# jlko/STOVE

Hardware: AMD Instinct MI355X
Metric: frames/s (fwd+bwd) for 3-obj billiards 32x32 T=100, 1/2/4/8 GPU; ELBO delta vs ref (higher is better)
Workload: dtype f32 (encoder GEMMs: fp32 products as 3 sixteen-bit MFMAs on hi/lo-split operands -- half pieces forward, bf16 pieces backward -- fp32 accumulate)

## Files before the change

### include/stove_hip.h

```cpp
#ifndef STOVE_HIP_H
#define STOVE_HIP_H
#include <stddef.h>
#include <stdint.h>

#ifdef __cplusplus
extern "C" {
#endif

int stove_abi_version(void);
const char* stove_error_string(int code);

typedef struct StoveSpnTables {
  const int32_t* obj_scope;
  const int32_t* obj_leaf_slot;
  const float* obj_coef;
  const float* obj_wsum;
  const float* obj_wroot;
  const int32_t* bg_side;
  const float* bg_coef;
  const float* bg_wroot;
  const float* bg_dense;
} StoveSpnTables;

size_t stove_bg_dense_floats(void);
// ... 255 lines not shown
int stove_supair_state_fwd2(const float* codes, const float* span_low, float* zc, float* pos, long long* idx, float* zfix,
                            unsigned char* hits, float* zl, float* sl, float* init, int init_ld, const float* lat_noise, int lat_dim,
                            int n, int T, int o, int skip, int fix, int mode, void* stream);
int stove_supair_state_bwd2(const float* zc, const long long* idx, const unsigned char* hits, const float* zfix, const float* g_zfix,
                            const float* g_zl, const float* g_sl, const float* g_init6, int init_ld, const float* span_low, float* gfix_ws,
                            float* g_codes, int n, int T, int o, int skip, void* stream);
int stove_zall_fwd(const float* zfix, const float* zs, float* zall, int n, int T, int o, int skip, void* stream);
int stove_zall_bwd(const float* zfix, const float* zs, const float* g_zall, const float* dz_in, float* g_zfix, float* g_zs, int n, int T, int o,
                   int skip, void* stream);
int stove_elbo_fwd(const float* zs, const float* mean, const float* std_, const float* zdyn, const float* lik, const float* trans_std16,
                   float* part_ws, float* out3, int n, int T, int o, int skip, void* stream);
int stove_elbo_bwd(const float* zs, const float* mean, const float* std_, const float* zdyn, const float* trans_std16, const float* g_out,
                   float* g_zs, float* g_mean, float* g_std, float* g_zdyn, float* g_lik, int n, int T, int o, int skip, void* stream);

void stove_debug_set_stamps(long long* device_buffer);

typedef struct StoveSpnArenaPlan {
  const int32_t* obj_mu;
  const int32_t* obj_rho;
  const int32_t* obj_sum;
  const int32_t* bg_mu;
  const int32_t* bg_rho;
  const int32_t* bg_gidx;
  int32_t obj_root, bg_root;
  float obj_vmin, obj_vmax, bg_vmin, bg_vmax;
} StoveSpnArenaPlan;
int stove_spn_bake(const float* arena, const StoveSpnArenaPlan* plan, float* obj_coef, float* obj_wsum, float* obj_wroot,
                   float* bg_coef, float* bg_wroot, void* stream);
int stove_spn_bake_bwd(const float* arena, const StoveSpnArenaPlan* plan, const StoveSpnTableGrads* g, float* grad_arena, void* stream);
int stove_arena_gather(const float* arena, const int32_t* src, float* image, int n, void* stream);
// ... 59 lines not shown
```

### stove_amd/_lib.py

```python
import ctypes
import os
from ctypes import POINTER, Structure, c_char_p, c_float, c_int, c_size_t, c_void_p

import torch

_HERE = os.path.dirname(os.path.abspath(__file__))
from . import settings as _settings

LIB_PATH = _settings.LIB_OVERRIDE or os.path.join(_HERE, 'libstove_hip.so')
_lib = None
ABI_VERSION = 7

class SpnTables(Structure):
    _fields_ = [('obj_scope', c_void_p), ('obj_leaf_slot', c_void_p), ('obj_coef', c_void_p),
                ('obj_wsum', c_void_p), ('obj_wroot', c_void_p),
                ('bg_side', c_void_p), ('bg_coef', c_void_p), ('bg_wroot', c_void_p), ('bg_dense', c_void_p)]


class SpnTableGrads(Structure):
    _fields_ = [('obj_coef', c_void_p), ('obj_wsum', c_void_p), ('obj_wroot', c_void_p),
                ('bg_coef', c_void_p), ('bg_wroot', c_void_p)]


class SpnArenaPlan(Structure):
# ... 85 lines not shown
        'stove_gnn_fwd_cl': (I, [P, P, P, P, I, I, I, I, I, I, P]),
        'stove_gnn_bwd_cl': (I, [P, P, P, P, P, P, P, I, I, I, I, I, I, P]),
        'stove_dynloop_fwd_cl': (I, [P] * 12 + [I] * 7 + [F] * 3 + [P]),
        'stove_dynloop_bwd_cl': (I, [P] * 18 + [I] * 7 + [F] * 3 + [P]),
        'stove_rollout_fwd_cl': (I, [P] * 6 + [I] * 8 + [F] * 3 + [P]),
        'stove_rollout_sample_fwd_cl': (I, [P] * 8 + [I] * 8 + [F] * 3 + [P]),
        'stove_match_objects': (I, [P, P, P, I, I, I, I, I, P]),
        'stove_profile_enable': (None, [I]),
        'stove_lstm_cell_fwd': (I, [P, P, P, P, P, I, I, I, P]),
        'stove_lstm_cell_bwd': (I, [P] * 10 + [I, I, I, I, P]),
        'stove_gnn_debug_stamps': (I, [P, P, P, P, P, P, I, I, I, I, I, P]),
        'stove_profile_report': (S, [c_char_p, S]),
        'stove_spn_bake': (I, [P, A, P, P, P, P, P, P]),
        'stove_spn_bake_bwd': (I, [P, A, G, P, P]),
        'stove_debug_set_stamps': (None, [P]),
        'stove_glimpse_mean': (I, [P, P, P, I, I, I, P]),
        'stove_objspn_mpe': (I, [T, P, P, P, P, P, I, P]),
        'stove_render_frames': (I, [P, P, I, P, P, I, I, P]),
        'stove_render_frames_any': (I, [P, P, I, P, P, P, P] + [I] * 8 + [P]),
        'stove_enc_head_fwd': (I, [P, P, P, P, P, P, P, I, I, I, I, I, I, P]),
        'stove_enc_head_bwd_ws_floats': (S, [I, I]),
        'stove_enc_head_bwd': (I, [P, P, P, P, P, P, P, P, P, P, I, P, I, I, I, I, I, P]),
        'stove_colsum2': (I, [P, P, P, I, P, I, I, P]),
        'stove_small_tn_ws_floats': (S, [I, I, I]),
        'stove_small_tn': (I, [P, P, P, P, I, I, I, P]),
        'stove_dynloop_bwd_ws_bytes_ts': (S, [I, I, I]),
        'stove_bw_transform': (I, [P, P, I, I, I, P]),
        'stove_bw_transform_u8': (I, [P, P, I, I, I, P]),
        'stove_stream_after': (I, [P, P]),
        'stove_small_linear': (I, [P, P, P, P, I, I, I, I, P]),
# ... 110 lines not shown
```

### stove_amd/csrc/capi.hip

```cpp
#include "../../include/stove_hip.h"
#include <algorithm>

#include "common.h"
#include <string.h>
#include <stdlib.h>
#include <math.h>
#include <atomic>
#include <type_traits>
#include "validate.h"
static_assert(stove_validate::kStoveInvalidValue == (int)hipErrorInvalidValue, "validate.h returns hipErrorInvalidValue");
#define STOVE_VALIDATE(expr)                      \
  do {                                            \
    const int v__ = stove_validate::expr;         \
    if (v__) return v__;                          \
  } while (0)
#include "spn_obj.hip"
#include "spn_obj_generic.hip"
#include "spn_bg.hip"
#include "spn_bg_generic.hip"
#include "scene.hip"
#include "scene_fused.hip"
#include "scene_colour.hip"
#include "gnn.hip"
#include "match.hip"
// ... 793 lines not shown
}

static long long* g_sm_stamps = nullptr;
void stove_debug_set_stamps(long long* device_buffer) { g_sm_stamps = device_buffer; }

size_t stove_dynloop_act_floats(int B, int Ts, int N) {
  const int g = gnn_group_for(B, N);
  const size_t blockwise = (size_t)stove_gnn_blocks(B, N) * Ts * gnn_act_floats(N, g);
  if (small_graph(N)) {
    const size_t streams = (size_t)B * sm_act2_floats(N, Ts);
    return streams > blockwise ? streams : blockwise;
  }
  return blockwise;
}

int stove_dynloop_fwd(const float* z1, const float* zsup, const float* zsstd, const float* eps, const float* extra,
                      const float* params, float* z, float* zdyn, float* zdstd, float* mean, float* std_, float* pred, float* act,
                      int B, int Ts, int N, int sin_dim, int lim_enc, int elu, float pos_var, float vel_std, float lat_std,
                      void* stream) {
  STOVE_VALIDATE(dynloop_fwd(z1, zsup, zsstd, eps, extra, params, z, zdyn, zdstd, mean, std_, B, Ts, N, sin_dim));
  if (B == 0 || Ts == 0) return 0;
  LoopConst kc{pos_var, vel_std, lat_std};
  if (small_graph(N)) {
    auto launch = [&](auto save, auto nmx, auto e, auto nt, auto stamp) {
      constexpr int NMX = decltype(nmx)::value;
      return STOVE_LAUNCH_LDS((dyn_loop_fwd_small_k<decltype(save)::value, NMX, decltype(e)::value, decltype(nt)::value, decltype(stamp)::value>),
                              dim3(B), dim3(64 * kSmWaves), SmShape<NMX>::kLdsFloats * sizeof(float), (hipStream_t)stream, z1, zsup, zsstd, eps,
                              extra, params, z, zdyn, zdstd, mean, std_, pred, act, B, Ts, N, sin_dim, lim_enc, elu, kc, g_sm_stamps, 0, Ts);
    };
    if (g_sm_stamps != nullptr && act != nullptr && !elu && N == 3)
      return launch(Int<2>{}, Int<4>{}, std::false_type{}, Int<3>{}, std::true_type{});
    auto run = [&](auto save) {
      return with_small_graph<true>(N, elu, true, [&](auto nmx, auto e, auto nt) { return launch(save, nmx, e, nt, std::false_type{}); });
    };
    return act != nullptr ? run(Int<2>{}) : run(Int<0>{});
  }
  const int G = gnn_group_for(B, N);
  return with_flag(elu, [&](auto e) {
    return with_flag(N == 6 && G == 1, [&](auto n6) {
      return STOVE_LAUNCH_LDS((dyn_loop_fwd_k<decltype(e)::value, decltype(n6)::value>), dim3(stove_gnn_blocks(B, N)), dim3(256), kGnnLdsBytes,
                              (hipStream_t)stream, z1, zsup, zsstd, eps, extra, params, z, zdyn, zdstd, mean, std_, pred, act, B, Ts, N, G,
                              sin_dim, lim_enc, elu, kc);
    });
// ... 19 lines not shown
                                   dextra, g_params, ws, B, Ts, N, sin_dim, lim_enc, elu, pos_var, vel_std, lat_std, stream, stream);
}

int stove_dynloop_bwd_overlap(const float* z1, const float* zsup, const float* zsstd, const float* eps, const float* extra,
                              const float* params, const float* z, const float* act, const float* dz, const float* dzdyn,
                              const float* dmean, const float* dstd, const float* dpred, float* dz1, float* dzsup, float* dzsstd,
                              float* dextra, float* g_params, void* ws, int B, int Ts, int N, int sin_dim, int lim_enc, int elu,
                              float pos_var, float vel_std, float lat_std, void* stream, void* param_stream) {
  STOVE_VALIDATE(dynloop_bwd(z1, zsup, zsstd, eps, extra, params, z, dz1, dzsup, dzsstd, dextra, g_params, ws, B, Ts, N, sin_dim));
  hipStream_t st = (hipStream_t)stream;
  hipStream_t sp = param_stream != nullptr ? (hipStream_t)param_stream : st;
  LoopConst kc{pos_var, vel_std, lat_std};
  if (small_bwd_path(N, act)) {
    float* gpart = (float*)ws;
    float* dy = gpart + (size_t)B * kGnnGrads;
    const bool head = dz != nullptr && dzdyn != nullptr && dmean != nullptr && dstd != nullptr && dpred == nullptr && sin_dim == 16 && lim_enc == 2;
    auto launch = [&](auto nmx, auto e, auto nt, auto hd, auto stamp) {
      constexpr int NMX = decltype(nmx)::value;
      return STOVE_LAUNCH_LDS((dyn_loop_bwd_small_k<NMX, decltype(e)::value, decltype(nt)::value, decltype(hd)::value, decltype(stamp)::value>),
                              dim3(B), dim3(64 * kSmWaves), smb_lds_floats<NMX>() * sizeof(float), st, zsup, zsstd, eps, params,
                              const_cast<float*>(act), dz, dzdyn, dmean, dstd, dpred, dz1, dzsup, dzsstd, dextra, dy, B, Ts, N, sin_dim, lim_enc,
                              elu, kc, g_sm_stamps, 0, Ts, (float*)nullptr);
    };
    int rc;
    if (g_sm_stamps != nullptr && !elu && N == 3 && head) {
      rc = launch(Int<4>{}, std::false_type{}, Int<3>{}, std::true_type{}, std::true_type{});
    } else {
      rc = with_small_graph<true>(N, elu, head, [&](auto nmx, auto e, auto nt) {
        constexpr int NT = decltype(nt)::value;
        if constexpr (NT == 6) {
          return launch(nmx, e, nt, std::true_type{}, std::false_type{});
        } else {
          if constexpr (NT == 3) {
            if (head) return launch(nmx, e, nt, std::true_type{}, std::false_type{});
          }
          return launch(nmx, e, nt, std::false_type{}, std::false_type{});
        }
      });
    }
    if (rc) return rc;
    STOVE_TRY(stream_after(sp, st));
    rc = STOVE_LAUNCH_LDS(gnn_dw_small_k, dim3(B), dim3(256), kDwLdsFloats * sizeof(float), sp, act, (const float*)dy, gpart, B, Ts, N);
    if (rc) return rc;
    STOVE_LAUNCH(reduce_chunks_k, dim3((kGnnGrads + 31) / 32), dim3(256), 0, sp, (const float*)gpart, g_params, kGnnGrads, B, 0);
    STOVE_LAUNCH_CHECK();
    return 0;
  }
  const int nb = stove_gnn_blocks(B, N), G = gnn_group_for(B, N);
  int rc = with_flag(elu, [&](auto e) {
    return with_flag(N == 6 && G == 1, [&](auto n6) {
      return STOVE_LAUNCH_LDS((dyn_loop_bwd_k<decltype(e)::value, decltype(n6)::value>), dim3(nb), dim3(256), kGnnLdsBytes, st, z1, zsup, zsstd,
                              eps, extra, params, z, act, dz, dzdyn, dmean, dstd, dpred, dz1, dzsup, dzsstd, dextra, (float*)ws, B, Ts, N, G,
                              sin_dim, lim_enc, elu, kc);
    });
  });
// ... 1136 lines not shown
```

### stove_amd/csrc/gnn_small.hip

```cpp
#include "common.h"
#include "split16.h"

namespace stove {

constexpr int kSmW = W_END;
constexpr int kSmWaves = 4;

template <int NMX>
struct SmShape {
  static_assert(NMX == 4 || NMX == 6, "built for up to four or up to six objects");
  static constexpr int RP = NMX > 4 ? 2 : 1;
  static constexpr int ET = (NMX * (NMX - 1) + 15) / 16;
  static constexpr int NE = NMX * NMX;
  static constexpr int kLdsFloats = kSmW + V_END + NMX * 256 + NMX * 4 + NE * 32 + ((NE + 3) & ~3);
};

struct SmLds {
  float *W, *V, *PR, *POS, *R3, *ATT;
};
template <int NMX>
__device__ __forceinline__ SmLds sm_carve(float* base) {
  SmLds L;
  L.W = base;
  L.V = L.W + kSmW;
// ... 487 lines not shown
    }
    sm_mfma_layer<2>(ws1, h1, acc);
    if (el[0].valid) {
#pragma unroll
      for (int t = 0; t < 2; ++t) {
        sm_st4(sdx + el[0].node32 + 16 * t, acc[t] + h1[t]);
        if (SAVE) sm_st4(act.H1 + el[0].node32 + 16 * t, h1[t]);
      }
    }
    return;
  }
  if ((wv != 2 && wv != 3) || cf.N < 2) return;
  sm_edge_chain<SAVE, ET>(L, cf, act, el, pre, cw, wv == 2 ? 1 : 0);
}

template <bool SAVE, int NMX>
__device__ __forceinline__ void sm_step(const SmLds& L, const SmCfg& cf, float sinv, const SmAct& act, float& res_out, float& pred_out,
                                        const SmEdgeLane (&el)[SmShape<NMX>::ET], const SmChainW& cw) {
  constexpr int RP = SmShape<NMX>::RP, ET = SmShape<NMX>::ET;
  constexpr bool HK = RP == 1;
  __shared__ __attribute__((aligned(16))) float sbuf[NMX][32];
  __shared__ __attribute__((aligned(16))) float sdx[NMX][32];
  const int wv = wave_id();
  const int lane = lane_id();
  const int o = lane & 31;
  const int N = cf.N;
  const int r = RP == 2 ? wv + 4 * (lane >> 5) : wv;
  const bool own = RP == 2 ? r < N : (lane < 32 && r < N);
  const int rs = r < N ? r : wv;
  const float* V = L.V;
  float S = 0.0f;
  SmW<8> wa, wb;
  sm_stamp(cf, 0);
// ... 7 lines not shown
      for (int g = 0; g < 4; ++g) ef[k4][g] = *reinterpret_cast<const float4*>(L.W + W_EF + (k4 * 256 + g * 64 + lane) * 4);
    float e;
    if (HK) {
      e = sm_dotw<8, HK>(wa, sinv);
    } else if (cf.sin_dim <= 16) {
      SmW<4> w4;
#pragma unroll
      for (int k4 = 0; k4 < 4; ++k4) w4.w[k4] = wa.w[k4];
      e = sm_dotw<4>(w4, sinv);
    } else {
      e = sm_dotw<8, HK>(wa, sinv);
    }
    S = (o < cf.lim_enc) ? sinv : e + benc;
    if (own) {
      sbuf[r][o] = S;
      if (SAVE) {
        act.SIN[r * 32 + o] = sinv;
        act.S[r * 32 + o] = S;
      }
      if (o < 2) L.POS[r * 4 + o] = S;
    }
#pragma unroll
    for (int rq = 0; rq < RP; ++rq) {
      const int row = wv + 4 * rq;
      if (rq > 0) {
        if (row >= N) break;
#pragma unroll
        for (int k4 = 0; k4 < 2; ++k4)
#pragma unroll
          for (int g = 0; g < 4; ++g) ef[k4][g] = *reinterpret_cast<const float4*>(L.W + W_EF + (k4 * 256 + g * 64 + lane) * 4);
      }
// ... 54 lines not shown
    sm_stamp(cf, 12);
    const float F1 = fast_tanh(sm_dotw<8, HK>(wa, pred) + bf0);
    sm_stamp(cf, 13);
    wa = sm_wload<8, HK>(L.W + W_F2, 32, o);
    const float F2 = fast_tanh(sm_dotw<8, HK>(wb, F1) + bf1) + F1;
    wb = sm_wload<8, HK>(L.W + W_O0, 32, o);
    const float F3 = sm_dotw<8, HK>(wa, F2) + bf2;
    wa = sm_wload<8, HK>(L.W + W_O0, 32, o, 8);
    float t = sm_dotw<8, HK>(wb, F3);
    wb = sm_wload<8, HK>(L.W + W_O1, 32, o);
    t += sm_dotw<8, HK>(wa, S);
    const float O1 = fast_tanh(t + bo0);
    sm_stamp(cf, 14);
    const float RES = sm_dotw<8, HK>(wb, O1) + bo1 + O1;
    sm_stamp(cf, 15);
    if (SAVE && own) {
      act.PRED[r * 32 + o] = pred;
      act.F1[r * 32 + o] = F1;
      act.F2[r * 32 + o] = F2;
      act.F3[r * 32 + o] = F3;
      act.O1[r * 32 + o] = O1;
      act.RES[r * 32 + o] = RES;
    }
    res_out = RES;
    pred_out = pred;
  }
  sm_stamp(cf, 6);
}

__device__ __forceinline__ float sm_from_lane(float v, int src_lane) {
  return __builtin_bit_cast(float, __builtin_amdgcn_ds_bpermute(src_lane * 4, __builtin_bit_cast(int, v)));
}

template <int SAVEM, int NMX, bool ELU, int NT, bool STAMP = false>
__global__ __launch_bounds__(64 * kSmWaves) void dyn_loop_fwd_small_k(
    const float* __restrict__ z1, const float* __restrict__ zsup, const float* __restrict__ zsstd,
    const float* __restrict__ eps, const float* __restrict__ extra, const float* __restrict__ P,
    float* __restrict__ z, float* __restrict__ zdyn, float* __restrict__ zdstd, float* __restrict__ mean,
    float* __restrict__ stdv, float* __restrict__ pred, float* __restrict__ act,
    int B, int Ts, int N, int sin_dim, int lim_enc, int elu, LoopConst kc, long long* stamps, int ts0, int ts1) {
  constexpr bool SAVE = SAVEM != 0;
  constexpr int RP = SmShape<NMX>::RP, ET = SmShape<NMX>::ET;
  static_assert(SAVEM == 0 || SAVEM == 2, "no saved activations, or the streams layout");
  static_assert(NT <= NMX, "object count beyond what the kernel is built for");
  if (!STAMP) stamps = nullptr;
  extern __shared__ __attribute__((aligned(16))) float lds[];
  const SmLds L = sm_carve<NMX>(lds);
  const int b = blockIdx.x;
  const int wv = wave_id(), lane = lane_id(), l = lane & 31;
  elu = ELU ? 1 : 0;
  if (NT > 0) N = NT;
  SmCfg cf{N, sin_dim, lim_enc, elu};
  cf.stamps = nullptr;
  const int E = sin_dim - 16;
  SmEdgeLane el[ET];
#pragma unroll
  for (int t = 0; t < ET; ++t) el[t] = sm_edge_lane(N, SAVE, t);
  sm_setup(L, P);
  float sinv = 0.0f;
  const int r = RP == 2 ? wv + 4 * (lane >> 5) : wv;
  const bool row = r < N;
  const bool own = RP == 2 ? row : (lane < 32 && row);
  if (row) {
    if (l < 16) sinv = ts0 == 0 ? z1[((size_t)b * N + r) * 18 + 2 + l] : z[(((size_t)b * Ts + ts0 - 1) * N + r) * 18 + 2 + l];
    else if (l < sin_dim) sinv = extra[(((size_t)b * Ts + ts0) * N + r) * E + (l - 16)];
  }
  WG_SYNC();
  SmChainW cw;
  sm_chain_wbuild(L, cw);
  for (int ts = ts0; ts < ts1; ++ts) {
    const size_t o = ((size_t)b * Ts + ts) * N + r;
    float ep = 0.0f, ms = 0.0f, ss = 1.0f, xnext = 0.0f;
    if (row) {
      if (l < 16) ep = eps[o * 18 + 2 + l];
      else if (l < 18) ep = eps[o * 18 + (l - 16)];
      if (l < 4) {
        ms = zsup[o * 6 + 2 + l];
        ss = zsstd[o * 6 + 2 + l];
      } else if (l >= 16 && l < 18) {
        ms = zsup[o * 6 + (l - 16)];
        ss = zsstd[o * 6 + (l - 16)];
      }
      if (l >= 16 && l < sin_dim && ts + 1 < Ts) xnext = extra[(((size_t)b * Ts + ts + 1) * N + r) * E + (l - 16)];
    }
    SmAct a{};
    if (SAVE) a = sm_act2(act + (size_t)b * sm_act2_floats(N, Ts), N, Ts, ts);
    cf.stamps = (ts == ts1 - 1) ? stamps : nullptr;
    float res = 0.0f, prd = 0.0f;
    sm_step<SAVE, NMX>(L, cf, sinv, a, res, prd, el, cw);
    if (wv < N) {
      const float res_s = from_xor16(res);
      float zv;
      if (l < 16) {
        const int d = l;
        const float m = 2.0f * __builtin_amdgcn_rcpf(1.0f + __expf(-res)) - 1.0f;
        const float sd = std_scale(d, kc) * __builtin_amdgcn_rcpf(1.0f + __expf(-res_s));
        const float zd = m + (d < 2 ? sinv : 0.0f);
        float mu, sg;
        if (d < 4) {
          const float sd2 = sd * sd, ss2 = ss * ss, D = sd2 + ss2;
          mu = (ss2 * zd + sd2 * ms) * __builtin_amdgcn_rcpf(D);
          sg = sd * ss * __builtin_amdgcn_rsqf(D);
        } else {
          mu = zd;
          sg = sd;
// ... 16 lines not shown
        }
      }
      if (pred != nullptr && own) pred[o * 32 + l] = prd;
      sinv = zv;
    }
    sm_stamp(cf, 7);
  }
}

template <int NMX, bool ELU, int NT>
__global__ __launch_bounds__(64 * kSmWaves) void rollout_fwd_small_k(const float* __restrict__ z_last, const float* __restrict__ extra,
                                                           const float* __restrict__ P, float* __restrict__ z_pred,
                                                           float* __restrict__ zstd, float* __restrict__ pred,
                                                           int B, int num, int A, int N, int sin_dim, int lim_enc, int elu, LoopConst kc) {
  constexpr int RP = SmShape<NMX>::RP, ET = SmShape<NMX>::ET;
  static_assert(NT <= NMX, "object count beyond what the kernel is built for");
  extern __shared__ __attribute__((aligned(16))) float lds[];
  const SmLds L = sm_carve<NMX>(lds);
  const int b = blockIdx.x;
  const int wv = wave_id(), lane = lane_id(), l = lane & 31;
  elu = ELU ? 1 : 0;
  if (NT > 0) N = NT;
  SmCfg cf{N, sin_dim, lim_enc, elu};
  cf.stamps = nullptr;
  const int E = sin_dim - 16;
  SmEdgeLane el[ET];
#pragma unroll
  for (int t = 0; t < ET; ++t) el[t] = sm_edge_lane(N, 0, t);
  sm_setup(L, P);
  float sinv = 0.0f, scale = 0.0f;
  const int r = RP == 2 ? wv + 4 * (lane >> 5) : wv;
  const bool row = r < N;
  const bool own = RP == 2 ? row : (lane < 32 && row);
  if (row) {
    if (l < 16) sinv = z_last[((size_t)b * N + r) * 18 + 2 + l];
    else if (l < sin_dim) sinv = extra[(((size_t)b * A + 0) * N + r) * E + (l - 16)];
    if (l >= 16 && l < 18) scale = z_last[((size_t)b * N + r) * 18 + (l - 16)];
  }
  WG_SYNC();
  SmChainW cw;
  sm_chain_wbuild(L, cw);
  for (int t = 0; t < num; ++t) {
    const size_t o = ((size_t)b * num + t) * N + r;
    float xnext = 0.0f;
    if (row && l >= 16 && l < sin_dim && t + 1 < num) xnext = extra[(((size_t)b * A + ((t + 1) % A)) * N + r) * E + (l - 16)];
    SmAct a{};
    float res = 0.0f, prd = 0.0f;
    sm_step<false, NMX>(L, cf, sinv, a, res, prd, el, cw);
    if (wv < N) {
      const float res_s = from_xor16(res);
      float zv;
      if (l < 16) {
        zv = 2.0f * sigmoidf_(res) - 1.0f + (l < 2 ? sinv : 0.0f);
        if (own) {
          z_pred[o * 18 + 2 + l] = zv;
          if (zstd != nullptr) zstd[o * 16 + l] = std_scale(l, kc) * sigmoidf_(res_s);
        }
      } else {
        zv = xnext;
        if (l < 18 && own) z_pred[o * 18 + (l - 16)] = scale;
      }
      if (pred != nullptr && own) pred[o * 32 + l] = prd;
      sinv = zv;
    }
  }
}

template <int NMX, bool ELU, int NT>
__global__ __launch_bounds__(64 * kSmWaves) void rollout_sample_fwd_small_k(const float* __restrict__ z_last, const float* __restrict__ extra,
                                                                  const float* __restrict__ P, const float* __restrict__ eps,
                                                                  float* __restrict__ z_pred, float* __restrict__ log_q,
                                                                  float* __restrict__ zstd, float* __restrict__ pred,
                                                                  int B, int num, int A, int N, int sin_dim, int lim_enc, int elu, LoopConst kc) {
  constexpr int RP = SmShape<NMX>::RP, ET = SmShape<NMX>::ET;
  static_assert(NT <= NMX, "object count beyond what the kernel is built for");
  extern __shared__ __attribute__((aligned(16))) float lds[];
  const SmLds L = sm_carve<NMX>(lds);
  const int b = blockIdx.x;
  const int wv = wave_id(), lane = lane_id(), l = lane & 31;
  elu = ELU ? 1 : 0;
  if (NT > 0) N = NT;
  SmCfg cf{N, sin_dim, lim_enc, elu};
  cf.stamps = nullptr;
  const int E = sin_dim - 16;
  SmEdgeLane el[ET];
#pragma unroll
  for (int t = 0; t < ET; ++t) el[t] = sm_edge_lane(N, 0, t);
  sm_setup(L, P);
  float sinv = 0.0f, scale = 0.0f;
  const int r = RP == 2 ? wv + 4 * (lane >> 5) : wv;
  const bool row = r < N;
  const bool own = RP == 2 ? row : (lane < 32 && row);
  if (row) {
    if (l < 16) sinv = z_last[((size_t)b * N + r) * 18 + 2 + l];
    else if (l < sin_dim) sinv = extra[(((size_t)b * A + 0) * N + r) * E + (l - 16)];
    if (l >= 16 && l < 18) scale = z_last[((size_t)b * N + r) * 18 + (l - 16)];
  }
  WG_SYNC();
  SmChainW cw;
  sm_chain_wbuild(L, cw);
  for (int t = 0; t < num; ++t) {
    const size_t o = ((size_t)b * num + t) * N + r;
    float xnext = 0.0f;
    if (row && l >= 16 && l < sin_dim && t + 1 < num) xnext = extra[(((size_t)b * A + ((t + 1) % A)) * N + r) * E + (l - 16)];
    const float ep = (row && l < 16) ? eps[o * 16 + l] : 0.0f;
    SmAct a{};
    float res = 0.0f, prd = 0.0f;
    sm_step<false, NMX>(L, cf, sinv, a, res, prd, el, cw);
    if (wv < N) {
      const float res_s = from_xor16(res);
      float zv;
      if (l < 16) {
        const float mean = 2.0f * sigmoidf_(res) - 1.0f + (l < 2 ? sinv : 0.0f);
        const float sd = std_scale(l, kc) * sigmoidf_(res_s);
        zv = fmaf(sd, ep, mean);
        if (own) {
          z_pred[o * 18 + 2 + l] = zv;
          log_q[o * 16 + l] = sample_log_q(ep, sd);
          if (zstd != nullptr) zstd[o * 16 + l] = sd;
        }
      } else {
        zv = xnext;
        if (l < 18 && own) z_pred[o * 18 + (l - 16)] = scale;
      }
// ... 8 lines not shown
```

### stove_amd/csrc/gnn_small_bwd.hip

```cpp
#include "common.h"

namespace stove {

struct SmDy {
  float *dRES, *dO1, *dF3, *duF1, *dF1p, *dSD, *dH1p, *dEnc, *dP, *dR3, *E32, *dA2p, *dR1p, *dA1p, *dq;
};
__host__ __device__ inline size_t sm_dy_floats(int N, int Ts) {
  const size_t f = (size_t)Ts * ((size_t)N * (8 * 32 + 256) + (size_t)N * (N - 1) * (3 * 32 + 2 * 64 + 1));
  return (f + 3) & ~(size_t)3;
}
__device__ __forceinline__ SmDy sm_dy(float* seq, int N, int Ts, int ts) {
  SmDy d;
  const size_t nrows = (size_t)Ts * N, erows = (size_t)Ts * N * (N - 1);
  float* nb = seq + (size_t)ts * N * 32;
  d.dRES = nb; d.dO1 = nb + nrows * 32; d.dF3 = nb + 2 * nrows * 32; d.duF1 = nb + 3 * nrows * 32; d.dF1p = nb + 4 * nrows * 32;
  d.dSD = nb + 5 * nrows * 32; d.dH1p = nb + 6 * nrows * 32; d.dEnc = nb + 7 * nrows * 32;
  d.dP = seq + nrows * 8 * 32 + (size_t)ts * N * 256;
  float* eb = seq + nrows * (8 * 32 + 256);
  const size_t eo = (size_t)ts * N * (N - 1);
  d.dR3 = eb + eo * 32; d.E32 = eb + erows * 32 + eo * 32; d.dA2p = eb + 2 * erows * 32 + eo * 32;
  float* e64 = eb + 3 * erows * 32;
  d.dR1p = e64 + eo * 64; d.dA1p = e64 + erows * 64 + eo * 64;
  d.dq = e64 + 2 * erows * 64 + eo;
  return d;
// ... 187 lines not shown
      }
      if (gq == 0) L.DD[dd_stride * h + el[c].e] = dd;
    }
  }
}

template <int NMX, bool ELU, int NT, bool HEAD, bool STAMP = false>
__global__ __launch_bounds__(64 * kSmWaves) void dyn_loop_bwd_small_k(
    const float* __restrict__ zsup, const float* __restrict__ zsstd, const float* __restrict__ eps, const float* __restrict__ P,
    float* __restrict__ act, const float* __restrict__ dz, const float* __restrict__ dzdyn, const float* __restrict__ dmean,
    const float* __restrict__ dstd, const float* __restrict__ dpred, float* __restrict__ dz1, float* __restrict__ dzsup,
    float* __restrict__ dzsstd, float* __restrict__ dextra, float* __restrict__ dy, int B, int Ts, int N, int sin_dim, int lim_enc,
    int elu, LoopConst kc, long long* stamps, int ts0, int ts1, float* __restrict__ carry) {
  constexpr int RP = SmShape<NMX>::RP, ET = SmShape<NMX>::ET, NE4 = (SmShape<NMX>::NE + 3) & ~3;
  constexpr bool HK = RP == 1;
  static_assert(NT <= NMX, "object count beyond what the kernel is built for");
  extern __shared__ __attribute__((aligned(16))) float lds[];
  __builtin_amdgcn_s_setprio(3);
  const SmBLds L = smb_carve<NMX>(lds);
  const int b = blockIdx.x;
  const int wv = wave_id(), lane = lane_id(), l = lane & 31, h = lane >> 5;
  elu = ELU ? 1 : 0;
  if (NT > 0) N = NT;
  if (!STAMP) stamps = nullptr;
  if (HEAD) {
    __builtin_assume(dz != nullptr);
    __builtin_assume(dzdyn != nullptr);
    __builtin_assume(dmean != nullptr);
    __builtin_assume(dstd != nullptr);
    dpred = nullptr;
// ... 13 lines not shown
  const int r = RP == 2 ? wv + 4 * h : wv;
  const bool row = r < N;
  const bool own = RP == 2 ? row : (lane < 32 && row);
  const int rs = row ? r : wv;
  const bool node = wv < N;
  float car = 0.0f;
  SmBNodeIn nin{};
  if (row) {
    const SmAct a = sm_act2(aseq, N, Ts, ts1 - 1);
    nin = smb_node_load(a, r, l, ((size_t)b * Ts + ts1 - 1) * N + r, eps, zsup, zsstd, dz, dzdyn, dmean, dstd, dpred);
    if (ts1 < Ts && l < 16) car = carry[((size_t)b * N + r) * 18 + 2 + l];
  }
  WG_SYNC();
  SmBChainW cw;
  smb_chain_wbuild(L, cw);
  for (int ts = ts1 - 1; ts >= ts0; --ts) {
    cf.stamps = (ts == ts0 + 1 && stamps != nullptr) ? stamps + 64 : nullptr;
    sm_stamp(cf, 0);
    const SmAct a = sm_act2(aseq, N, Ts, ts);
    const SmDy g = sm_dy(dseq, N, Ts, ts);
    const size_t o = ((size_t)b * Ts + ts) * N + r;
    const SmBNodeIn cur = nin;
    if (row && ts > ts0) {
      const SmAct an = sm_act2(aseq, N, Ts, ts - 1);
      nin = smb_node_load(an, r, l, o - N, eps, zsup, zsstd, dz, dzdyn, dmean, dstd, dpred);
    }
    SmBEdgeIn ein[ET] = {};
    if (wv >= 2) {
#pragma unroll
      for (int t = 0; t < ET; ++t) ein[t] = smb_edge_load(a, el[t], wv == 2 ? 1 : 0);
    }
    float* pos = L.POS + (ts & 1) * (NMX * 4);
    float dS_o0 = 0.0f, dSD = 0.0f, pc = 0.0f;
    if (node) {
      SmW<8> wa = sm_wload<8, HK>(L.W + W_O1, 32, l), wb;
      if (l < 2 && own) pos[r * 4 + l] = cur.S;
      const float res_hi = from_xor16(cur.RES);
      const float gz = cur.gz + (l < 16 ? car : 0.0f);
      const float gmu = gz + cur.gmu_in, gsg = gz * cur.ep + cur.gsg_in;
      float lo = 0.0f, hi = 0.0f;
      if (l < 16) {
        const int d = l;
        const float kd = std_scale(d, kc);
        const float m = 2.0f * __builtin_amdgcn_rcpf(1.0f + __expf(-cur.RES)) - 1.0f;
        const float sg_hi = __builtin_amdgcn_rcpf(1.0f + __expf(-res_hi));
        const float sd = kd * sg_hi;
        const float zd = m + (d < 2 ? cur.SIN : 0.0f);
        float gzd = cur.gzd_in, gsd;
        if (d < 4) {
          const float ms = cur.ms, ss = cur.ss;
          const float sd2 = sd * sd, ss2 = ss * ss, D = sd2 + ss2, iD = __builtin_amdgcn_rcpf(D);
          const float mu = (ss2 * zd + sd2 * ms) * iD;
          const float rD = rsqrtf(D);
          gzd += gmu * ss2 * iD;
          gsd = gmu * (ms - mu) * iD * 2.0f * sd + gsg * ss * ss2 * iD * rD;
          if (own) {
            dzsup[o * 6 + 2 + d] = gmu * sd2 * iD;
            dzsstd[o * 6 + 2 + d] = gmu * (zd - mu) * iD * 2.0f * ss + gsg * sd * sd2 * iD * rD;
          }
        } else {
          gzd += gmu;
          gsd = gsg;
        }
        if (d < 2) pc = gzd;
        lo = gzd * 0.5f * (1.0f - m * m);
        hi = gsd * sd * (1.0f - sg_hi);
      } else if (l < 18 && own) {
        dzsup[o * 6 + (l - 16)] = gmu;
        dzsstd[o * 6 + (l - 16)] = gsg;
      }
      const float hi_from = from_xor16(hi);
      const float dres = l < 16 ? lo : hi_from;
      sm_stamp(cf, 6);
      wb = sm_wload<8, HK>(L.W + W_O0, 64, l);
      const float db = (sm_dotw<8, HK>(wa, dres) + dres) * (1.0f - cur.O1 * cur.O1);
      wa = sm_wload<8, HK>(L.W + W_O0, 64, 32 + l);
      const float dF3 = sm_dotw<8, HK>(wb, db);
      wb = sm_wload<8, HK>(L.W + W_F2, 32, l);
      dS_o0 = sm_dotw<8, HK>(wa, db);
      wa = sm_wload<8, HK>(L.W + W_F1, 32, l);
      const float dF2 = sm_dotw<8, HK>(wb, dF3);
      const float th = cur.F2 - cur.F1;
      const float du = dF2 * (1.0f - th * th);
      wb = sm_wload<8, HK>(L.W + W_F0, 32, l);
      const float dbf = (sm_dotw<8, HK>(wa, du) + dF2) * (1.0f - cur.F1 * cur.F1);
      dSD = sm_dotw<8, HK>(wb, dbf) + cur.dpred;
      if (own) {
        L.DSD[r * 32 + l] = dSD;
        g.dRES[r * 32 + l] = dres;
        g.dO1[r * 32 + l] = db;
        g.dF3[r * 32 + l] = dF3;
        g.duF1[r * 32 + l] = du;
        g.dF1p[r * 32 + l] = dbf;
        g.dSD[r * 32 + l] = dSD;
      }
    }
    sm_stamp(cf, 1);
    WG_SYNC();
    sm_stamp(cf, 2);
    smb_edge_phase_mfma<ET>(L, el, ein, g, elu, NE4, cw);
    sm_stamp(cf, 3);
    WG_SYNC();
    sm_stamp(cf, 4);
    if (node) {
      float dS_edge = 0.0f;
#pragma unroll
      for (int rq = 0; rq < RP; ++rq) {
        const int rw = wv + 4 * rq;
        if (rq > 0 && rw >= N) break;
        float dp[4] = {0.0f, 0.0f, 0.0f, 0.0f};
        for (int j = 0; j < N; ++j) {
          if (j == rw) continue;
          const float* e1 = L.EG + (rw * N + j) * 128;
          const float* e2 = L.EG + (j * N + rw) * 128;
          dp[0] += e1[lane];
          dp[1] += e2[lane];
          dp[2] += e1[64 + lane];
          dp[3] += e2[64 + lane];
        }
        float* dpr = L.DP + rw * 256;
#pragma unroll
        for (int gq = 0; gq < 4; ++gq) {
          dpr[lane + 64 * gq] = dp[gq];
          g.dP[rw * 256 + lane + 64 * gq] = dp[gq];
        }
        sm_stamp(cf, 7);
        v2f s0 = {0.0f, 0.0f}, s1 = {0.0f, 0.0f};
#pragma unroll
        for (int q = 0; q < 4; ++q) {
          float4 w[8], x[8];
#pragma unroll
          for (int u = 0; u < 8; ++u) {
            w[u] = *reinterpret_cast<const float4*>(L.W + W_EF + ((32 * h + 8 * q + u) * 32 + l) * 4);
            x[u] = *reinterpret_cast<const float4*>(dpr + 128 * h + 4 * (8 * q + u));
          }
#pragma unroll
          for (int u = 0; u < 8; ++u) {
            s0 = pk_fma(v2f{w[u].x, w[u].y}, v2f{x[u].x, x[u].y}, s0);
            s1 = pk_fma(v2f{w[u].z, w[u].w}, v2f{x[u].z, x[u].w}, s1);
// ... 7 lines not shown
      sm_stamp(cf, 8);
      SmW<8> wa = sm_wload<8, HK>(L.W + W_S1, 32, l);
      SmW<8> wb = sm_wload<8, HK>(L.W + W_S0, 32, l);
      const float dH1p = (sm_dotw<8, HK>(wa, dSD) + dSD) * dphi_from_out(cur.H1, elu);
      wa = sm_wload<8, HK>(L.W + W_ENC, 32, l);
      float tot = sm_dotw<8, HK>(wb, dH1p) + dS_edge + dS_o0;
      if (l < 2) {
        float dd = 0.0f;
        for (int j = 0; j < N; ++j)
          if (j != rs) dd += 2.0f * (pos[rs * 4 + l] - pos[j * 4 + l]) * ((L.DD[rs * N + j] + L.DD[NE4 + rs * N + j]) + (L.DD[j * N + rs] + L.DD[NE4 + j * N + rs]));
        tot += dd;
      }
      const bool raw = l < lim_enc;
      const float dEnc = raw ? 0.0f : tot;
      const float dsin = sm_dotw<8, HK>(wa, dEnc) + (raw ? tot : 0.0f);
      if (own) {
        g.dH1p[r * 32 + l] = dH1p;
        g.dEnc[r * 32 + l] = dEnc;
        if (l >= 16 && l < sin_dim) dextra[o * E + (l - 16)] = dsin;
      }
      car = (l < 16) ? dsin + (l < 2 ? pc : 0.0f) : 0.0f;
    }
    sm_stamp(cf, 5);
  }
  if (node) {
    const float shifted = sm_from_lane(car, (lane + 62) & 63);
    float* dst = ts0 == 0 ? dz1 : carry;
    if (l < 18 && own) dst[((size_t)b * N + r) * 18 + l] = l < 2 ? 0.0f : shifted;
  }
}

struct DwLds {
  float *SIN, *H1, *PRED, *F1, *F2, *O1, *CAT;
  float *dEnc, *dH1p, *dSD, *dF1p, *duF1, *dF3, *dO1, *dRES, *dP;
  float *R1, *A1, *dR1p, *dA1p;
  float *R2, *A2, *E32, *dA2p, *dR3;
// ... 140 lines not shown
```

### stove_amd/csrc/ppo_model.hip

```cpp
#include "common.h"
#include "ppo_policy.h"

namespace stove {

constexpr int kPmObsFloats = 32, kPmHeadFloats = 16, kPmEmbRows = 4 * env_step::kMaxObjects;
constexpr int kPmRhV = 104;
constexpr int kPmFloats = kPmObsFloats + 2 * ppo_policy::kMaxWidth + kPmHeadFloats + env_step::kMaxObjects * 32 +
                          kPmEmbRows * ppo_policy::kActions + kPmEmbRows + 1024 + 1024 + 512 + 128 + kPmRhV + 32 + 4;
constexpr size_t kPmStaticBytes = 4096;
constexpr size_t kPmLdsLimit = 160 * 1024;
static_assert(4 * env_step::kMaxObjects <= kPmObsFloats && ppo_policy::kHeads <= kPmHeadFloats, "the rows hold the widest case");
static_assert(ppo_policy::kMaxWidth <= 64 * kSmWaves, "a layer's neurons have a thread each");
static_assert(kPmFloats % 4 == 0, "the image behind it stays 16-byte aligned");

struct PmLds {
  float *o, *a, *b, *heads, *pred, *embw, *embb, *Wt0a, *Wt0b, *Wt1a, *Wt1b, *V, *xs, *img;
  int* act;
};
__device__ __forceinline__ PmLds pm_carve(float* base) {
  PmLds M;
  M.o = base;
  M.a = M.o + kPmObsFloats;
  M.b = M.a + ppo_policy::kMaxWidth;
  M.heads = M.b + ppo_policy::kMaxWidth;
// ... 132 lines not shown
    }
    __syncthreads();
    if (row && l >= 16) {
      if (l < 20) {
        const int action = M.act[0], o = r * 4 + (l - 16);
        float v = M.embb[o];
        for (int k = 0; k < ppo_policy::kActions; ++k) v = fmaf(k == action ? 1.0f : 0.0f, M.embw[o * ppo_policy::kActions + k], v);
        sinv = v;
      } else {
        sinv = appv;
      }
    }
    const size_t o = ((size_t)b * S + t) * N + r;
    SmAct a{};
    float res = 0.0f, prd = 0.0f;
    sm_step<false, NMX>(L, cf, sinv, a, res, prd, el, cw);
    if (wv < N) {
      float zv = 0.0f;
      if (l < 16) {
        zv = 2.0f * sigmoidf_(res) - 1.0f + (l < 2 ? sinv : 0.0f);
        if (own) z_pred[o * 18 + 2 + l] = zv;
      } else if (l < 18 && own) {
        z_pred[o * 18 + (l - 16)] = scale;
      }
      if (own) {
        if (pred != nullptr) pred[o * 32 + l] = prd;
        M.pred[r * 32 + l] = prd;
      }
      sinv = zv;
    }
  }
// ... 140 lines not shown
```

Measured before the change: 9.053 million.

## Defer global stores in small GNN dynamics loop to end of each step

For the NMX==4 small-graph kernels (forward, rollout, backward), activation and gradient stores are buffered in registers and issued together at the end of each timestep, after an explicit vmcnt wait. The goal is to keep scattered global writes and their waitcnt stalls out of the serial recurrent critical path. A debug hook is also added that lets the dynloop fwd/bwd run only a timestep slice with a carry buffer, with the backward weight-gradient pass skipped for non-initial pieces. The trade-off is more register pressure and full memory waits at step boundaries.

```diff
diff --git a/include/stove_hip.h b/include/stove_hip.h
--- a/include/stove_hip.h
+++ b/include/stove_hip.h
@@ -293,6 +293,7 @@
                    float* g_zs, float* g_mean, float* g_std, float* g_zdyn, float* g_lik, int n, int T, int o, int skip, void* stream);
 
 void stove_debug_set_stamps(long long* device_buffer);
+void stove_debug_set_piece(int ts0, int ts1, float* carry);
 
 typedef struct StoveSpnArenaPlan {
   const int32_t* obj_mu;
diff --git a/stove_amd/_lib.py b/stove_amd/_lib.py
--- a/stove_amd/_lib.py
+++ b/stove_amd/_lib.py
@@ -123,6 +123,7 @@
         'stove_spn_bake': (I, [P, A, P, P, P, P, P, P]),
         'stove_spn_bake_bwd': (I, [P, A, G, P, P]),
         'stove_debug_set_stamps': (None, [P]),
+        'stove_debug_set_piece': (None, [I, I, P]),
         'stove_glimpse_mean': (I, [P, P, P, I, I, I, P]),
         'stove_objspn_mpe': (I, [T, P, P, P, P, P, I, P]),
         'stove_render_frames': (I, [P, P, I, P, P, I, I, P]),
diff --git a/stove_amd/csrc/capi.hip b/stove_amd/csrc/capi.hip
--- a/stove_amd/csrc/capi.hip
+++ b/stove_amd/csrc/capi.hip
@@ -831,6 +831,18 @@
   return blockwise;
 }
 
+static int g_sm_ts0 = 0, g_sm_ts1 = 0;
+static float* g_sm_carry = nullptr;
+void stove_debug_set_piece(int ts0, int ts1, float* carry) {
+  g_sm_ts0 = ts0;
+  g_sm_ts1 = ts1;
+  g_sm_carry = carry;
+}
+static bool sm_piece(int Ts, int& p0, int& p1) {
+  p0 = g_sm_ts1 > 0 ? g_sm_ts0 : 0;
+  p1 = g_sm_ts1 > 0 ? g_sm_ts1 : Ts;
+  return p0 >= 0 && p0 < p1 && p1 <= Ts;
+}
 int stove_dynloop_fwd(const float* z1, const float* zsup, const float* zsstd, const float* eps, const float* extra,
                       const float* params, float* z, float* zdyn, float* zdstd, float* mean, float* std_, float* pred, float* act,
                       int B, int Ts, int N, int sin_dim, int lim_enc, int elu, float pos_var, float vel_std, float lat_std,
@@ -839,11 +851,13 @@
   if (B == 0 || Ts == 0) return 0;
   LoopConst kc{pos_var, vel_std, lat_std};
   if (small_graph(N)) {
+    int p0, p1;
+    if (!sm_piece(Ts, p0, p1)) return (int)hipErrorInvalidValue;
     auto launch = [&](auto save, auto nmx, auto e, auto nt, auto stamp) {
       constexpr int NMX = decltype(nmx)::value;
       return STOVE_LAUNCH_LDS((dyn_loop_fwd_small_k<decltype(save)::value, NMX, decltype(e)::value, decltype(nt)::value, decltype(stamp)::value>),
                               dim3(B), dim3(64 * kSmWaves), SmShape<NMX>::kLdsFloats * sizeof(float), (hipStream_t)stream, z1, zsup, zsstd, eps,
-                              extra, params, z, zdyn, zdstd, mean, std_, pred, act, B, Ts, N, sin_dim, lim_enc, elu, kc, g_sm_stamps, 0, Ts);
+                              extra, params, z, zdyn, zdstd, mean, std_, pred, act, B, Ts, N, sin_dim, lim_enc, elu, kc, g_sm_stamps, p0, p1);
     };
     if (g_sm_stamps != nullptr && act != nullptr && !elu && N == 3)
       return launch(Int<2>{}, Int<4>{}, std::false_type{}, Int<3>{}, std::true_type{});
@@ -893,13 +907,16 @@
   if (small_bwd_path(N, act)) {
     float* gpart = (float*)ws;
     float* dy = gpart + (size_t)B * kGnnGrads;
+    int p0, p1;
+    if (!sm_piece(Ts, p0, p1) || ((p0 > 0 || p1 < Ts) && g_sm_carry == nullptr)) return (int)hipErrorInvalidValue;
+    float* carry = g_sm_carry;
     const bool head = dz != nullptr && dzdyn != nullptr && dmean != nullptr && dstd != nullptr && dpred == nullptr && sin_dim == 16 && lim_enc == 2;
     auto launch = [&](auto nmx, auto e, auto nt, auto hd, auto stamp) {
       constexpr int NMX = decltype(nmx)::value;
       return STOVE_LAUNCH_LDS((dyn_loop_bwd_small_k<NMX, decltype(e)::value, decltype(nt)::value, decltype(hd)::value, decltype(stamp)::value>),
                               dim3(B), dim3(64 * kSmWaves), smb_lds_floats<NMX>() * sizeof(float), st, zsup, zsstd, eps, params,
                               const_cast<float*>(act), dz, dzdyn, dmean, dstd, dpred, dz1, dzsup, dzsstd, dextra, dy, B, Ts, N, sin_dim, lim_enc,
-                              elu, kc, g_sm_stamps, 0, Ts, (float*)nullptr);
+                              elu, kc, g_sm_stamps, p0, p1, carry);
     };
     int rc;
     if (g_sm_stamps != nullptr && !elu && N == 3 && head) {
@@ -918,6 +935,7 @@
       });
     }
     if (rc) return rc;
+    if (p0 > 0) return 0;
     STOVE_TRY(stream_after(sp, st));
     rc = STOVE_LAUNCH_LDS(gnn_dw_small_k, dim3(B), dim3(256), kDwLdsFloats * sizeof(float), sp, act, (const float*)dy, gpart, B, Ts, N);
     if (rc) return rc;
diff --git a/stove_amd/csrc/gnn_small.hip b/stove_amd/csrc/gnn_small.hip
--- a/stove_amd/csrc/gnn_small.hip
+++ b/stove_amd/csrc/gnn_small.hip
@@ -525,9 +525,14 @@
   sm_edge_chain<SAVE, ET>(L, cf, act, el, pre, cw, wv == 2 ? 1 : 0);
 }
 
-template <bool SAVE, int NMX>
+__device__ __forceinline__ void sm_wait_vm() { __builtin_amdgcn_s_waitcnt(0x0f70); }
+struct SmNodeOut {
+  float S, F1, F2, F3, O1;
+};
+
+template <bool SAVE, int NMX, bool DEFER = false>
 __device__ __forceinline__ void sm_step(const SmLds& L, const SmCfg& cf, float sinv, const SmAct& act, float& res_out, float& pred_out,
-                                        const SmEdgeLane (&el)[SmShape<NMX>::ET], const SmChainW& cw) {
+                                        const SmEdgeLane (&el)[SmShape<NMX>::ET], const SmChainW& cw, SmNodeOut& no) {
   constexpr int RP = SmShape<NMX>::RP, ET = SmShape<NMX>::ET;
   constexpr bool HK = RP == 1;
   __shared__ __attribute__((aligned(16))) float sbuf[NMX][32];
@@ -565,7 +570,7 @@
     S = (o < cf.lim_enc) ? sinv : e + benc;
     if (own) {
       sbuf[r][o] = S;
-      if (SAVE) {
+      if (SAVE && !DEFER) {
         act.SIN[r * 32 + o] = sinv;
         act.S[r * 32 + o] = S;
       }
@@ -650,7 +655,8 @@
     sm_stamp(cf, 14);
     const float RES = sm_dotw<8, HK>(wb, O1) + bo1 + O1;
     sm_stamp(cf, 15);
-    if (SAVE && own) {
+    if (DEFER) no = SmNodeOut{S, F1, F2, F3, O1};
+    if (SAVE && !DEFER && own) {
       act.PRED[r * 32 + o] = pred;
       act.F1[r * 32 + o] = F1;
       act.F2[r * 32 + o] = F2;
@@ -676,6 +682,7 @@
     float* __restrict__ stdv, float* __restrict__ pred, float* __restrict__ act,
     int B, int Ts, int N, int sin_dim, int lim_enc, int elu, LoopConst kc, long long* stamps, int ts0, int ts1) {
   constexpr bool SAVE = SAVEM != 0;
+  constexpr bool DEFER = NMX == 4;
   constexpr int RP = SmShape<NMX>::RP, ET = SmShape<NMX>::ET;
   static_assert(SAVEM == 0 || SAVEM == 2, "no saved activations, or the streams layout");
   static_assert(NT <= NMX, "object count beyond what the kernel is built for");
@@ -704,6 +711,7 @@
   WG_SYNC();
   SmChainW cw;
   sm_chain_wbuild(L, cw);
+  if (DEFER) sm_wait_vm();
   for (int ts = ts0; ts < ts1; ++ts) {
     const size_t o = ((size_t)b * Ts + ts) * N + r;
     float ep = 0.0f, ms = 0.0f, ss = 1.0f, xnext = 0.0f;
@@ -723,8 +731,59 @@
     if (SAVE) a = sm_act2(act + (size_t)b * sm_act2_floats(N, Ts), N, Ts, ts);
     cf.stamps = (ts == ts1 - 1) ? stamps : nullptr;
     float res = 0.0f, prd = 0.0f;
-    sm_step<SAVE, NMX>(L, cf, sinv, a, res, prd, el, cw);
-    if (wv < N) {
+    SmNodeOut no{};
+    sm_step<SAVE, NMX, DEFER>(L, cf, sinv, a, res, prd, el, cw, no);
+    if (DEFER) sm_wait_vm();
+    if (DEFER && wv < N) {
+      const float res_s = from_xor16(res);
+      float zv, zd = 0.0f, sd = 0.0f, mu, sg;
+      if (l < 16) {
+        const int d = l;
+        const float m = 2.0f * __builtin_amdgcn_rcpf(1.0f + __expf(-res)) - 1.0f;
+        sd = std_scale(d, kc) * __builtin_amdgcn_rcpf(1.0f + __expf(-res_s));
+        zd = m + (d < 2 ? sinv : 0.0f);
+        if (d < 4) {
+          const float sd2 = sd * sd, ss2 = ss * ss, D = sd2 + ss2;
+          mu = (ss2 * zd + sd2 * ms) * __builtin_amdgcn_rcpf(D);
+          sg = sd * ss * __builtin_amdgcn_rsqf(D);
+        } else {
+          mu = zd;
+          sg = sd;
+        }
+        zv = fmaf(sg, ep, mu);
+      } else {
+        zv = xnext;
+        mu = ms;
+        sg = ss;
+      }
+      if (own) {
+        if (l < 16) {
+          zdyn[o * 16 + l] = zd;
+          zdstd[o * 16 + l] = sd;
+          z[o * 18 + 2 + l] = zv;
+          mean[o * 18 + 2 + l] = mu;
+          stdv[o * 18 + 2 + l] = sg;
+        } else if (l < 18) {
+          const int q = l - 16;
+          z[o * 18 + q] = fmaf(ss, ep, ms);
+          mean[o * 18 + q] = mu;
+          stdv[o * 18 + q] = sg;
+        }
+        if (pred != nullptr) pred[o * 32 + l] = prd;
+        if (SAVE) {
+          a.SIN[r * 32 + l] = sinv;
+          a.S[r * 32 + l] = no.S;
+          a.PRED[r * 32 + l] = prd;
+          a.F1[r * 32 + l] = no.F1;
+          a.F2[r * 32 + l] = no.F2;
+          a.F3[r * 32 + l] = no.F3;
+          a.O1[r * 32 + l] = no.O1;
+          a.RES[r * 32 + l] = res;
+        }
+      }
+      sinv = zv;
+    }
+    if (!DEFER && wv < N) {
       const float res_s = from_xor16(res);
       float zv;
       if (l < 16) {
@@ -771,6 +830,7 @@
                                                            float* __restrict__ zstd, float* __restrict__ pred,
                                                            int B, int num, int A, int N, int sin_dim, int lim_enc, int elu, LoopConst kc) {
   constexpr int RP = SmShape<NMX>::RP, ET = SmShape<NMX>::ET;
+  constexpr bool DEFER = NMX == 4;
   static_assert(NT <= NMX, "object count beyond what the kernel is built for");
   extern __shared__ __attribute__((aligned(16))) float lds[];
   const SmLds L = sm_carve<NMX>(lds);
@@ -797,14 +857,37 @@
   WG_SYNC();
   SmChainW cw;
   sm_chain_wbuild(L, cw);
+  if (DEFER) sm_wait_vm();
   for (int t = 0; t < num; ++t) {
     const size_t o = ((size_t)b * num + t) * N + r;
     float xnext = 0.0f;
     if (row && l >= 16 && l < sin_dim && t + 1 < num) xnext = extra[(((size_t)b * A + ((t + 1) % A)) * N + r) * E + (l - 16)];
     SmAct a{};
     float res = 0.0f, prd = 0.0f;
-    sm_step<false, NMX>(L, cf, sinv, a, res, prd, el, cw);
-    if (wv < N) {
+    SmNodeOut no{};
+    sm_step<false, NMX>(L, cf, sinv, a, res, prd, el, cw, no);
+    if (DEFER) sm_wait_vm();
+    if (DEFER && wv < N) {
+      const float res_s = from_xor16(res);
+      float zv, sd = 0.0f;
+      if (l < 16) {
+        zv = 2.0f * sigmoidf_(res) - 1.0f + (l < 2 ? sinv : 0.0f);
+        if (zstd != nullptr) sd = std_scale(l, kc) * sigmoidf_(res_s);
+      } else {
+        zv = xnext;
+      }
+      if (own) {
+        if (l < 16) {
+          z_pred[o * 18 + 2 + l] = zv;
+          if (zstd != nullptr) zstd[o * 16 + l] = sd;
+        } else if (l < 18) {
+          z_pred[o * 18 + (l - 16)] = scale;
+        }
+        if (pred != nullptr) pred[o * 32 + l] = prd;
+      }
+      sinv = zv;
+    }
+    if (!DEFER && wv < N) {
       const float res_s = from_xor16(res);
       float zv;
       if (l < 16) {
@@ -830,6 +913,7 @@
                                                                   float* __restrict__ zstd, float* __restrict__ pred,
                                                                   int B, int num, int A, int N, int sin_dim, int lim_enc, int elu, LoopConst kc) {
   constexpr int RP = SmShape<NMX>::RP, ET = SmShape<NMX>::ET;
+  constexpr bool DEFER = NMX == 4;
   static_assert(NT <= NMX, "object count beyond what the kernel is built for");
   extern __shared__ __attribute__((aligned(16))) float lds[];
   const SmLds L = sm_carve<NMX>(lds);
@@ -856,6 +940,7 @@
   WG_SYNC();
   SmChainW cw;
   sm_chain_wbuild(L, cw);
+  if (DEFER) sm_wait_vm();
   for (int t = 0; t < num; ++t) {
     const size_t o = ((size_t)b * num + t) * N + r;
     float xnext = 0.0f;
@@ -863,8 +948,33 @@
     const float ep = (row && l < 16) ? eps[o * 16 + l] : 0.0f;
     SmAct a{};
     float res = 0.0f, prd = 0.0f;
-    sm_step<false, NMX>(L, cf, sinv, a, res, prd, el, cw);
-    if (wv < N) {
+    SmNodeOut no{};
+    sm_step<false, NMX>(L, cf, sinv, a, res, prd, el, cw, no);
+    if (DEFER) sm_wait_vm();
+    if (DEFER && wv < N) {
+      const float res_s = from_xor16(res);
+      float zv, sd = 0.0f, lq = 0.0f;
+      if (l < 16) {
+        const float mean = 2.0f * sigmoidf_(res) - 1.0f + (l < 2 ? sinv : 0.0f);
+        sd = std_scale(l, kc) * sigmoidf_(res_s);
+        zv = fmaf(sd, ep, mean);
+        lq = sample_log_q(ep, sd);
+      } else {
+        zv = xnext;
+      }
+      if (own) {
+        if (l < 16) {
+          z_pred[o * 18 + 2 + l] = zv;
+          log_q[o * 16 + l] = lq;
+          if (zstd != nullptr) zstd[o * 16 + l] = sd;
+        } else if (l < 18) {
+          z_pred[o * 18 + (l - 16)] = scale;
+        }
+        if (pred != nullptr) pred[o * 32 + l] = prd;
+      }
+      sinv = zv;
+    }
+    if (!DEFER && wv < N) {
       const float res_s = from_xor16(res);
       float zv;
       if (l < 16) {
diff --git a/stove_amd/csrc/gnn_small_bwd.hip b/stove_amd/csrc/gnn_small_bwd.hip
--- a/stove_amd/csrc/gnn_small_bwd.hip
+++ b/stove_amd/csrc/gnn_small_bwd.hip
@@ -225,6 +225,7 @@
     int elu, LoopConst kc, long long* stamps, int ts0, int ts1, float* __restrict__ carry) {
   constexpr int RP = SmShape<NMX>::RP, ET = SmShape<NMX>::ET, NE4 = (SmShape<NMX>::NE + 3) & ~3;
   constexpr bool HK = RP == 1;
+  constexpr bool DEFER = NMX == 4;
   static_assert(NT <= NMX, "object count beyond what the kernel is built for");
   extern __shared__ __attribute__((aligned(16))) float lds[];
   __builtin_amdgcn_s_setprio(3);
@@ -268,6 +269,7 @@
   WG_SYNC();
   SmBChainW cw;
   smb_chain_wbuild(L, cw);
+  if (DEFER) sm_wait_vm();
   for (int ts = ts1 - 1; ts >= ts0; --ts) {
     cf.stamps = (ts == ts0 + 1 && stamps != nullptr) ? stamps + 64 : nullptr;
     sm_stamp(cf, 0);
@@ -286,6 +288,8 @@
     }
     float* pos = L.POS + (ts & 1) * (NMX * 4);
     float dS_o0 = 0.0f, dSD = 0.0f, pc = 0.0f;
+    float gsup = 0.0f, gsstd = 0.0f, q_dres = 0.0f, q_db = 0.0f, q_dF3 = 0.0f, q_du = 0.0f, q_dbf = 0.0f;
+    float q_dp[4] = {0.0f, 0.0f, 0.0f, 0.0f}, q_dH1p = 0.0f, q_dEnc = 0.0f, q_dsin = 0.0f;
     if (node) {
       SmW<8> wa = sm_wload<8, HK>(L.W + W_O1, 32, l), wb;
       if (l < 2 && own) pos[r * 4 + l] = cur.S;
@@ -308,7 +312,11 @@
           const float rD = rsqrtf(D);
           gzd += gmu * ss2 * iD;
           gsd = gmu * (ms - mu) * iD * 2.0f * sd + gsg * ss * ss2 * iD * rD;
-          if (own) {
+          if (DEFER) {
+#pragma clang fp contract(off)
+            gsup = gmu * sd2 * iD;
+            gsstd = gmu * (zd - mu) * iD * 2.0f * ss + gsg * sd * sd2 * iD * rD;
+          } else if (own) {
             dzsup[o * 6 + 2 + d] = gmu * sd2 * iD;
             dzsstd[o * 6 + 2 + d] = gmu * (zd - mu) * iD * 2.0f * ss + gsg * sd * sd2 * iD * rD;
           }
@@ -319,6 +327,9 @@
         if (d < 2) pc = gzd;
         lo = gzd * 0.5f * (1.0f - m * m);
         hi = gsd * sd * (1.0f - sg_hi);
+      } else if (DEFER) {
+        gsup = gmu;
+        gsstd = gsg;
       } else if (l < 18 && own) {
         dzsup[o * 6 + (l - 16)] = gmu;
         dzsstd[o * 6 + (l - 16)] = gsg;
@@ -339,7 +350,10 @@
       wb = sm_wload<8, HK>(L.W + W_F0, 32, l);
       const float dbf = (sm_dotw<8, HK>(wa, du) + dF2) * (1.0f - cur.F1 * cur.F1);
       dSD = sm_dotw<8, HK>(wb, dbf) + cur.dpred;
-      if (own) {
+      if (DEFER) {
+        if (own) L.DSD[r * 32 + l] = dSD;
+        q_dres = dres; q_db = db; q_dF3 = dF3; q_du = du; q_dbf = dbf;
+      } else if (own) {
         L.DSD[r * 32 + l] = dSD;
         g.dRES[r * 32 + l] = dres;
         g.dO1[r * 32 + l] = db;
@@ -352,6 +366,7 @@
     sm_stamp(cf, 1);
     WG_SYNC();
     sm_stamp(cf, 2);
+    if (DEFER) sm_wait_vm();
     smb_edge_phase_mfma<ET>(L, el, ein, g, elu, NE4, cw);
     sm_stamp(cf, 3);
     WG_SYNC();
@@ -376,7 +391,8 @@
 #pragma unroll
         for (int gq = 0; gq < 4; ++gq) {
           dpr[lane + 64 * gq] = dp[gq];
-          g.dP[rw * 256 + lane + 64 * gq] = dp[gq];
+          if (DEFER) q_dp[gq] = dp[gq];
+          else g.dP[rw * 256 + lane + 64 * gq] = dp[gq];
         }
         sm_stamp(cf, 7);
         v2f s0 = {0.0f, 0.0f}, s1 = {0.0f, 0.0f};
@@ -414,12 +430,39 @@
       const bool raw = l < lim_enc;
       const float dEnc = raw ? 0.0f : tot;
       const float dsin = sm_dotw<8, HK>(wa, dEnc) + (raw ? tot : 0.0f);
-      if (own) {
+      if (DEFER) {
+        q_dH1p = dH1p; q_dEnc = dEnc; q_dsin = dsin;
+      } else if (own) {
         g.dH1p[r * 32 + l] = dH1p;
         g.dEnc[r * 32 + l] = dEnc;
         if (l >= 16 && l < sin_dim) dextra[o * E + (l - 16)] = dsin;
       }
       car = (l < 16) ? dsin + (l < 2 ? pc : 0.0f) : 0.0f;
+    }
+    if (DEFER) {
+      sm_wait_vm();
+      if (node && own) {
+        if (l < 4) {
+          dzsup[o * 6 + 2 + l] = gsup;
+          dzsstd[o * 6 + 2 + l] = gsstd;
+        } else if (l >= 16 && l < 18) {
+          dzsup[o * 6 + (l - 16)] = gsup;
+          dzsstd[o * 6 + (l - 16)] = gsstd;
+        }
+        g.dRES[r * 32 + l] = q_dres;
+        g.dO1[r * 32 + l] = q_db;
+        g.dF3[r * 32 + l] = q_dF3;
+        g.duF1[r * 32 + l] = q_du;
+        g.dF1p[r * 32 + l] = q_dbf;
+        g.dSD[r * 32 + l] = dSD;
+        g.dH1p[r * 32 + l] = q_dH1p;
+        g.dEnc[r * 32 + l] = q_dEnc;
+        if (l >= 16 && l < sin_dim) dextra[o * E + (l - 16)] = q_dsin;
+      }
+      if (node) {
+#pragma unroll
+        for (int gq = 0; gq < 4; ++gq) g.dP[wv * 256 + lane + 64 * gq] = q_dp[gq];
+      }
     }
     sm_stamp(cf, 5);
   }
diff --git a/stove_amd/csrc/ppo_model.hip b/stove_amd/csrc/ppo_model.hip
--- a/stove_amd/csrc/ppo_model.hip
+++ b/stove_amd/csrc/ppo_model.hip
@@ -170,7 +170,8 @@
     const size_t o = ((size_t)b * S + t) * N + r;
     SmAct a{};
     float res = 0.0f, prd = 0.0f;
-    sm_step<false, NMX>(L, cf, sinv, a, res, prd, el, cw);
+    SmNodeOut no{};
+    sm_step<false, NMX>(L, cf, sinv, a, res, prd, el, cw, no);
     if (wv < N) {
       float zv = 0.0f;
       if (l < 16) {
```

Measured after the change: 9.188 million (median of 6 runs). 1.5% higher.
